# Renmusxd/RustQIP

Measured on AMD Instinct MI355X. Metric: single-qubit gate apply GB/s (algorithmic bytes: 32 * 2^n per H / X / Rz gate), higher is better.
Workload: dtype f64; 1 GPU; 256 random single-qubit gates (uniform H / X / Rz(theta), uniform target; configs[1] generator, seed 28, single-qubit part) at n=30 (30 qubits = 16 GiB per GPU), Complex<f64>, resident non-uniform state; n_qubits=30, n_local=30, parallelism=single GPU

## Files before the change

### rustqip_amd/build.py

```python
from __future__ import annotations

import os
import subprocess
import sys

HERE = os.path.dirname(os.path.abspath(__file__))
CSRC = os.path.join(HERE, "csrc")
UNITS = ["qip_core", "qip_launch", "qip_tile_sched", "qip_circuit", "qip_tile_interp", "qip_jit", "qip_slice", "qip_host", "qip_measure", "qip_dist"]
HEADERS = [os.path.join(CSRC, h) for h in ("qip_kernels.h", "qip_internal.h", "qip_jit.h", "qip_tile.h")] + [
    os.path.join(HERE, "..", "include", "qip_hip.h"), os.path.join(HERE, "..", "include", "qip_hip_debug.h"),
    os.path.join(HERE, "..", "include", "qip_hipx.h")]
OBJDIR = os.path.join(HERE, "build")
OUT = os.path.join(HERE, "lib", "libqip_hip.so")
JITC = os.path.join(HERE, "lib", "qip_jitc")
JITC_SRC = os.path.join(CSRC, "qip_jitc.c")
HIPCC = os.environ.get("HIPCC", "/opt/rocm/bin/hipcc")
FLAGS = ["--offload-arch=gfx950", "-O3", "-std=c++17", "-ffp-contract=off", "-fno-slp-vectorize", "-fPIC"]
if os.environ.get("QIP_HIP_TUNING"):
    FLAGS.append("-DQIP_HIP_TUNING")
UNIT_FLAGS = {"qip_tile_interp": ["-mllvm", "-structurizecfg-skip-uniform-regions"]}
LINK = ["--offload-arch=gfx950", "-fPIC", "-shared", "-Wl,--version-script=" + os.path.join(CSRC, "exports.map")]
LIBS = ["-ldl"]

EMBED = os.path.join(CSRC, "qip_kernels_embed.inc")


def write_embed() -> None:
    with open(HEADERS[0]) as f:
        text = f.read()
    assert ')QIPKSRC"' not in text
    body = 'R"QIPKSRC(' + text + ')QIPKSRC"\n'
    if not os.path.exists(EMBED) or open(EMBED).read() != body:
# ... 50 lines not shown
```

### rustqip_amd/csrc/qip_circuit.hip

```cpp
#include "qip_tile.h"

typedef std::complex<double> cd;
struct Cluster {
  std::vector<uint32_t> pos;
  std::vector<cd> m;
};

template <typename T>
static bool op_to_dense(uint32_t n, const FlatOp& f, uint32_t max_k, std::vector<uint32_t>* pos,
                        std::vector<cd>* mat) {
  if (!f.distinct || f.k_all > max_k) return false;
  const uint32_t kt = f.k_all, k = f.n_op;
  const size_t S = (size_t)1 << kt, Si = (size_t)1 << k, thr = S - Si;
  pos->clear();
  for (uint32_t j = 0; j < kt; ++j) pos->push_back(n - 1 - (uint32_t)f.outer->indices[j]);
  mat->assign(S * S, cd(0, 0));
  for (size_t r = 0; r < thr; ++r) (*mat)[r * S + r] = cd(1, 0);
  const T* dense = static_cast<const T*>(f.inner->dense);
  const T* vals = static_cast<const T*>(f.inner->sparse_vals);
  for (size_t r = 0; r < Si; ++r) {
    switch (f.inner->kind) {
      case QIP_OP_MATRIX:
        for (size_t c = 0; c < Si; ++c)
          (*mat)[(thr + r) * S + thr + c] = cd(dense[2 * (r * Si + c)], dense[2 * (r * Si + c) + 1]);
// ... 696 lines not shown
  if (run.prepare()) return QIP_OK;
  if (!params.empty()) QCHK(arena_upload(s, params.data(), params.size() * sizeof(T), 0));
  ProfRec rec;
  rec.cls = KC_TILE_GATES;
  if (s->profile) QCHK(prof_begin(s, KC_TILE_GATES, sweep_bytes, &rec));
  void* st_ptr = s->cur;
  uint64_t second_arg = ntiles;
  void* params_ptr = s->arena;
  void* out_ptr = s->alt;
  void* args_p[] = {&st_ptr, &second_arg, &params_ptr, &out_ptr};
  void* args_np[] = {&st_ptr, &second_arg, &out_ptr};
  void** args = (parametrised || !f.folding) ? args_p : args_np;
  const dim3 grid = grid2d(ntiles >> (f.sl ? f.sl->nbits : 0), 1);
  return run_parts(s, run, f, &rec, [&](uint32_t k) -> int {
    if (f.sl) second_arg = f.slice_or(k);
    return jit_run(s, job, [&](hipFunction_t fn) -> int {
      HIPCHK(hipModuleLaunchKernel(fn, grid.x, grid.y, 1, block, 1, 1, (unsigned)lds, s->stream, args, nullptr));
      return QIP_OK;
    });
  });
}

template <typename T>
static int launch_tile_segment(qip_hip_state* s, const BatchRun& run, const std::vector<const TileItem*>& seg,
                               std::vector<uint32_t> high_in, const TileStorePerm* fold = nullptr, TileSlicing* sl = nullptr,
                               uint32_t p5_override = 0, const std::vector<uint32_t>* grid_ctl = nullptr, double alg_bytes = 0) {
  arena_begin_group(s);
  TileSegmentPlan<T> plan;
  TileAbsorbedX absorbed;
  if (s->tile_passes && !run.tile_jit && !grid_ctl && !p5_override)
    QCHK(build_tile_segment_absorbed<T>(s->n, seg, std::move(high_in), &plan, run.tile >= 2 ? 2 : 1, &absorbed));
  else
    QCHK(build_tile_segment<T>(s->n, s->tile_passes != 0, seg, std::move(high_in), &plan, run.tile >= 2 ? 2 : 1, p5_override));
  const std::vector<uint32_t>& high = plan.high;
  TileInterpPlan<T> interp;
  if (!s->tile_passes && !plan.diags.empty()) return fail(QIP_ERR_INVALID, "internal: a multi-qubit diagonal item in a k_tile_gates segment");
  const bool use_runs = (g_tile_diag_runs || !plan.diags.empty()) && s->tile_passes && !run.tile_jit;
  if (use_runs) tile_merge_diag_runs<T>(plan, &interp, g_tile_diag_runs ? 2u : ~0u);
  const bool has_runs = use_runs && interp.runs > 0;
  std::vector<TileGate<T>>& gates = has_runs ? interp.gates : plan.gates;
  std::vector<amp_t<T>>& mats = plan.mats;
  TilePassDesc& pd = has_runs ? interp.pd : plan.pd;
  const size_t gates_bytes = gates.size() * sizeof(TileGate<T>);
  const size_t mats_bytes = mats.size() * sizeof(amp_t<T>);
  const size_t items_bytes = has_runs ? interp.items.size() * sizeof(TileDiagItem<T>) : 0;
  static_assert(sizeof(TileGate<T>) % 16 == 0, "the matrix block behind the gate list stays 16-byte aligned");
  static_assert(sizeof(amp_t<T>) * 16 % 16 == 0 && sizeof(TileDiagItem<T>) % 16 == 0, "... and the diagonal steps behind the matrices");
  const size_t items_off = (gates_bytes + mats_bytes + 15) / 16 * 16;
  auto upload_gates = [&]() -> int {
    QCHK(ensure_arena(s, items_off + items_bytes));
    QCHK(arena_upload(s, gates.data(), gates_bytes, 0));
    if (!mats.empty()) QCHK(arena_upload(s, mats.data(), mats_bytes, gates_bytes));
    if (items_bytes) QCHK(arena_upload(s, interp.items.data(), items_bytes, items_off));
    return QIP_OK;
  };
  TileDesc d;
  memset(&d, 0, sizeof d);
  d.ngates = (uint32_t)gates.size();
  for (int j = 0; j < kTileHigh; ++j) d.hpos[j] = high[j];
  d.p5 = plan.p5;
  Ins ins = tile_ins(high, plan.p5);
  uint64_t ntiles = 1ull << (s->n - kTileBits);
  const bool whole_grid = !grid_ctl || grid_ctl->empty();
  if (!whole_grid) {
    uint64_t ones = 0;
    for (uint32_t c : *grid_ctl) ones |= 1ull << (c == 5u ? plan.p5 : c);
    ins = tile_ins(high, plan.p5, *grid_ctl, ones);
    ntiles >>= grid_ctl->size();
  }
  const double sweep_bytes = alg_bytes > 0 ? alg_bytes : 2.0 * (double)s->amp_bytes * (double)s->namps;
  TileSweep f;
  QCHK(plan_sweep(s, run, fold, sl, s->tile_passes && whole_grid, kTileBits, high, plan.p5, &ins, &f));
  const size_t lds = sizeof(amp_t<T>) << kTileBits;
  if (s->tile_passes && run.tile_jit) {
    const bool fma = s->tile_fma && run.tile >= 2;
    const bool parametrised = run.tile_jit != 3;
// ... 2 lines not shown
    int remap = ntiles % 64 == 0 ? (int)g_tile_remap : 0;
    if (remap == 4) {
      uint32_t nb = 0, J = 0;
      while ((1ull << nb) < ntiles) ++nb;
      uint32_t seen = 0;
      for (uint32_t pp = kTileLow; pp < s->n && seen < nb; ++pp) {
        bool opened = false;
        for (uint32_t j = 0; j < ins.npos; ++j) opened = opened || ins.pos[j] == pp;
        if (opened) continue;
        if (pp < 16) ++J;
        ++seen;
      }
      if (nb < 3) remap = 0;
      else remap = 16 + (int)std::min(J, nb - 3);
    }
    if (f.sl) remap = 0;
    const std::string src = tile_jit_source<T>(plan, ins, use_nt(s), remap, parametrised ? &params : nullptr, merge, f.folding ? fold : nullptr, f.sl != nullptr);
    return launch_compiled<T>(s, run, f, src, fma, parametrised, params, ntiles, kTileBlock, lds, sweep_bytes);
  }
  if (run.prepare()) return QIP_OK;
  QCHK(upload_gates());
  const TileGate<T>* dg = (const TileGate<T>*)s->arena;
  const amp_t<T>* dmats = (const amp_t<T>*)((const char*)s->arena + gates_bytes);
  const TileDiagItem<T>* ditems = (const TileDiagItem<T>*)((const char*)s->arena + items_off);
  ProfRec rec;
  rec.cls = KC_TILE_GATES;
  if (s->profile) QCHK(prof_begin(s, KC_TILE_GATES, sweep_bytes, &rec));
  if (s->tile_passes) {
    const uint64_t ntiles_part = ntiles >> (f.sl ? f.sl->nbits : 0);
    return run_parts(s, run, f, &rec, [&](uint32_t k) -> int {
      Ins ins_k = ins;
      ins_k.ormask |= f.slice_or(k);
      launch_tile_passes<T>(s->stream, grid2d(ntiles_part, 1), lds, use_nt(s), (amp_t<T>*)s->cur, ins_k, pd, dg, dmats, (amp_t<T>*)s->alt,
                            f.folding ? fold : nullptr, ditems);
      HIPCHK(hipGetLastError());
      return QIP_OK;
    });
  }
  if (use_nt(s))
    hipLaunchKernelGGL((k_tile_gates<T, true>), grid2d(ntiles, 1), dim3(kBlock), lds, s->stream, (amp_t<T>*)s->cur, ins, d, dg);
  else
    hipLaunchKernelGGL((k_tile_gates<T, false>), grid2d(ntiles, 1), dim3(kBlock), lds, s->stream, (amp_t<T>*)s->cur, ins, d, dg);
  HIPCHK(hipGetLastError());
  if (s->profile) QCHK(prof_end(s, &rec));
  return QIP_OK;
}

template <typename T>
static int launch_wide_segment(qip_hip_state* s, const BatchRun& run, const std::vector<const TileItem*>& seg, std::vector<uint32_t> high_in,
                               const TileStorePerm* fold = nullptr, TileSlicing* sl = nullptr) {
  arena_begin_group(s);
  WidePlan<T> plan;
  QCHK(build_wide_segment<T>(s->n, seg, std::move(high_in), &plan, run.tile >= 2 ? 2 : 1));
  Ins ins = tile_ins(plan.high, plan.p5);
  TileSweep f;
  QCHK(plan_sweep(s, run, fold, sl, true, kWideBits, plan.high, plan.p5, &ins, &f));
// ... 681 lines not shown
```

### rustqip_amd/csrc/qip_kernels.h

```cpp
#pragma once

#ifndef __HIPCC_RTC__
#include <hip/hip_runtime.h>
#include <stdint.h>
#else
typedef __hip_internal::uint32_t uint32_t;
typedef __hip_internal::uint64_t uint64_t;
typedef __hip_internal::int32_t int32_t;
typedef __hip_internal::int64_t int64_t;
#endif

namespace qipk {

constexpr int kBlock = 256;
constexpr int kMaxIns = 64;

template <typename T> struct V2;
template <> struct V2<double> { using type = double __attribute__((ext_vector_type(2))); };
template <> struct V2<float> { using type = float __attribute__((ext_vector_type(2))); };
template <typename T> using amp_t = typename V2<T>::type;
template <typename A, typename B> struct SameT { static constexpr bool v = false; };
template <typename A> struct SameT<A, A> { static constexpr bool v = true; };
template <int V> struct IntC { static constexpr int v = V; };


struct Ins {
  uint64_t ormask;
  uint32_t npos;
  uint32_t pos[kMaxIns];
};

template <int NP>
// ... 1408 lines not shown
  for (int i = 0; i < NE; ++i) {
    if ((i >> J) & 1) continue;
    const int k = i | (1 << J);
    const A a0 = e[i], a1 = e[k];
    const T p0x = m0 * a0.x, p0y = m0 * a0.y, p1x = m1 * a1.x, p1y = m1 * a1.y;
    e[i].x = p0x + p1x;
    e[i].y = p0y + p1y;
    e[k].x = tile_signed_sum<N0, N1>(p0x, p1x);
    e[k].y = tile_signed_sum<N0, N1>(p0y, p1y);
    __builtin_amdgcn_sched_barrier(0);
  }
}

template <typename T, int J, int NE>
__device__ __forceinline__ void pass_dense_signs(const TileGate<T>& g, amp_t<T> (&e)[NE]) {
  switch (g.b1 & (kTileSignNeg0 | kTileSignNeg1)) {
    case 0u: pass_dense_signs_body<T, J, false, false, NE>(g, e); break;
    case kTileSignNeg1: pass_dense_signs_body<T, J, false, true, NE>(g, e); break;
    case kTileSignNeg0: pass_dense_signs_body<T, J, true, false, NE>(g, e); break;
    default: pass_dense_signs_body<T, J, true, true, NE>(g, e); break;
  }
}

template <typename T, int J, int NE, bool LOOP = false>
__device__ __forceinline__ void pass_dense(const TileGate<T>& g, amp_t<T> (&e)[NE], const uint32_t (&c)[NE], uint32_t cm) {
  using A = amp_t<T>;
  const bool is_x = (g.b1 & 2u) != 0, real = (g.b1 & 1u) != 0;
  if (is_x) {
#pragma unroll
    for (int i = 0; i < NE; ++i) {
      if ((i >> J) & 1) continue;
      const int k = i | (1 << J);
      if ((c[i] & cm) != cm) continue;
      QIP_KEEP_BRANCH();
      if constexpr (LOOP) {
        cswap_inplace(e[i], e[k]);
      } else {
        const A a0 = e[i];
        e[i] = e[k];
        e[k] = a0;
      }
    }
    return;
  }
  if (cm == 0u && real && (g.b1 & kTileSignRows) != 0) {
    QIP_KEEP_BRANCH();
    pass_dense_signs<T, J, NE>(g, e);
  } else if (cm == 0u && g.nz == 15u) {
    if (real) pass_dense_body<T, J, true, false, NE, LOOP>(g, e, c, cm);
    else pass_dense_body<T, J, false, false, NE, LOOP>(g, e, c, cm);
  } else {
    if (real) pass_dense_body<T, J, true, true, NE, LOOP>(g, e, c, cm);
    else pass_dense_body<T, J, false, true, NE, LOOP>(g, e, c, cm);
  }
}

template <typename T, int J, int NE>
__device__ __forceinline__ void pass_dense_lane(const TileGate<T>& g, amp_t<T> (&e)[NE], const uint32_t (&c)[NE], uint32_t cm,
                                                bool lane_ok) {
  using A = amp_t<T>;
  const bool h0 = (g.nz & 1u) != 0, h1 = (g.nz & 2u) != 0, h2 = (g.nz & 4u) != 0, h3 = (g.nz & 8u) != 0;
#pragma unroll
  for (int i = 0; i < NE; ++i) {
    if ((i >> J) & 1) continue;
    const int k = i | (1 << J);
    if ((c[i] & cm) != cm) continue;
    QIP_KEEP_BRANCH();
    const A a0 = e[i], a1 = e[k];
// ... 99 lines not shown
    if (((base >> JA) & 1) || ((base >> JB) & 1) || ((base >> JC) & 1)) continue;
    if ((c[base] & cm) != cm) continue;
    QIP_KEEP_BRANCH();
    A x[8];
#pragma unroll
    for (int s = 0; s < 8; ++s) x[s] = e[base | (((s >> 2) & 1) << JA) | (((s >> 1) & 1) << JB) | ((s & 1) << JC)];
#pragma unroll
    for (int r = 0; r < 8; ++r) {
      A acc = cmul(M[r * 8], x[0]);
#pragma unroll
      for (int s = 1; s < 8; ++s) acc = cadd(acc, cmul(M[r * 8 + s], x[s]));
      const int i = base | (((r >> 2) & 1) << JA) | (((r >> 1) & 1) << JB) | ((r & 1) << JC);
      e[i] = lane_ctl ? tile_sel(lane_ok, acc, x[r]) : acc;
      __builtin_amdgcn_sched_barrier(0);
    }
  }
}
template <typename T, int JA, int JB, int JC>
__device__ __forceinline__ void pass_dense3(const amp_t<T>* __restrict__ M, amp_t<T> (&e)[8], bool lane_ctl, bool lane_ok) {
  const uint32_t c0[8] = {0, 0, 0, 0, 0, 0, 0, 0};
  pass_dense3w<T, JA, JB, JC, 8>(M, e, c0, 0u, lane_ctl, lane_ok);
}

template <typename T, bool NT, bool FOLD = false>
__global__ __launch_bounds__(kTileBlock, 5) void k_tile_passes(amp_t<T>* __restrict__ st, Ins ins, TilePassDesc d,
                                                                              const TileGate<T>* __restrict__ gates,
                                                                              const amp_t<T>* __restrict__ mats,
                                                                              amp_t<T>* __restrict__ out = nullptr,
                                                                              TileStorePerm sp = TileStorePerm(),
                                                                              const TileDiagItem<T>* __restrict__ diag = nullptr) {
  using A = amp_t<T>;
  extern __shared__ __attribute__((aligned(16))) unsigned char tile_raw[];
  A* tile = reinterpret_cast<A*>(tile_raw);
  constexpr int PER = (1 << kTileBits) / kTileBlock;
  static_assert(PER == 8 && kTileLow == 6, "tile index = (u << kTileLaneBits) | (wave << 6) | lane");
  const uint32_t tid = threadIdx.x;
  const uint32_t lane = tid & 63u;
  const uint32_t wave = __builtin_amdgcn_readfirstlane(tid >> 6);
  uint64_t wbase = tile_block_base(blockIdx.x + (uint64_t)blockIdx.y * gridDim.x, ins, d.p5);
  const uint64_t base = wbase;
#pragma unroll
  for (int j = 0; j < kTileWaveBits; ++j) wbase |= (uint64_t)((wave >> j) & 1u) << d.hpos[j];
  const uint32_t slot_tid = tile_slot<A>(tid);
  const uint32_t lane_off = tile_lane_off(lane, d.p5);
  {
    A x[PER];
#pragma unroll
    for (int u = 0; u < PER; ++u) {
      const uint64_t ub = wbase | ((uint64_t)(u & 1) << d.hpos[kTileWaveBits]) | ((uint64_t)((u >> 1) & 1) << d.hpos[kTileWaveBits + 1]) |
                          ((uint64_t)((u >> 2) & 1) << d.hpos[kTileWaveBits + 2]);
      x[u] = ldg<NT>(st + ub + lane_off);
    }
#pragma unroll
    for (int u = 0; u < PER; ++u) tile[slot_tid ^ tile_slot<A>((uint32_t)u << kTileLaneBits)] = x[u];
  }
  __syncthreads();
  for (uint32_t pi = 0; pi < d.npasses; ++pi) {
    const TilePass ps = d.pass[pi];
    uint32_t tb = 0;
    const uint32_t lp_lo = (uint32_t)ps.lanepos, lp_hi = (uint32_t)(ps.lanepos >> 32);
#pragma unroll
    for (int k = 0; k < kTileLaneBits; ++k) tb |= ((tid >> k) & 1u) << (((k < 8 ? lp_lo : lp_hi) >> (4 * (k & 7))) & 15u);
    const uint32_t slot_tb = tile_slot<A>(tb);
    uint32_t c[8];
    A e[8];
#pragma unroll
    for (int i = 0; i < 8; ++i) {
      c[i] = ((uint32_t)(i & 1) << ps.pb[0]) | ((uint32_t)((i >> 1) & 1) << ps.pb[1]) |
             ((uint32_t)((i >> 2) & 1) << ps.pb[2]);
      e[i] = tile[slot_tb ^ tile_slot<A>(c[i])];
    }
    const TileGate<T>* gp = gates + ps.first;
    const TileGate<T>* const gend = gp + ps.count;
    for (; gp != gend; ++gp) {
      const TileGate<T> g = *gp;
      if ((base & g.omask) != g.omask) continue;
      const uint32_t cm_reg = g.cm_reg;
      switch (g.op) {
        case TOP_DIAG_RUN: {
          const TileDiagItem<T>* ip = diag + g.nz;
          const TileDiagItem<T>* const iend = ip + g.b1;
#ifndef QIP_DIAG_PREFETCH
#define QIP_DIAG_PREFETCH 0
#endif
#ifndef QIP_DIAG_ASM
#define QIP_DIAG_ASM 1
#endif
#if QIP_DIAG_PREFETCH
          TileDiagItem<T> nxt = *ip;
#endif
          for (; ip != iend;) {
#if QIP_DIAG_PREFETCH
            const TileDiagItem<T> it = nxt;
            ++ip;
            if (ip != iend) nxt = *ip;
#else
            const TileDiagItem<T> it = *ip;
            ++ip;
#endif
            if ((base & it.omask) != it.oval) continue;
            A f = it.f1;
            const uint32_t selp = it.emask_sel >> 24;
            if (selp != 0u) {
              QIP_KEEP_BRANCH();
              f = tile_sel(((tb >> (selp - 1u)) & 1u) != 0u, it.f1, it.f0);
            }
            if (it.lane_mask != 0u) {
              QIP_KEEP_BRANCH();
              const bool lane_ok = (tb & it.lane_mask) == it.lane_val;
              f.x = lane_ok ? f.x : (T)1;
              f.y = lane_ok ? f.y : (T)0;
            }
#pragma unroll
            for (int i = 0; i < 8; ++i)
              if ((it.emask_sel >> i) & 1u) {
                QIP_KEEP_BRANCH();
#if QIP_DIAG_ASM
                cscale_inplace(f, e[i]);
#else
                e[i] = cmul(f, e[i]);
#endif
              }
          }
          break;
        }
        case TOP_DIAG_UNIFORM: {
          const A f = ((base >> g.tpos_out) & 1ull) ? g.m[1] : g.m[0];
          if (f.x == (T)1 && f.y == (T)0) break;
          QIP_KEEP_BRANCH();
          pass_scale<T, 0, -1, 8, true>(f, e, c, cm_reg);
          break;
        }
        case TOP_DIAG_LANE:
        case TOP_DIAG_LANE_CTL: {
          const bool outside = g.b0 == kTileOutside;
          const bool one = outside ? ((base >> g.tpos_out) & 1ull) != 0 : ((tb >> g.b0) & 1u) != 0;
          A f = tile_sel(one, g.m[1], g.m[0]);
          if (g.op == TOP_DIAG_LANE_CTL) {
            QIP_KEEP_BRANCH();
            const bool lane_ok = (tb & g.cm_lane) == g.cm_lane;
            f.x = lane_ok ? f.x : (T)1;
            f.y = lane_ok ? f.y : (T)0;
          }
          pass_scale<T, 0, -1, 8, true>(f, e, c, cm_reg);
          break;
        }
        case TOP_DIAG_REG0: pass_diag<T, 0, 8, true>(g, e, c, cm_reg, g.cm_lane != 0u, (tb & g.cm_lane) == g.cm_lane); break;
        case TOP_DIAG_REG1: pass_diag<T, 1, 8, true>(g, e, c, cm_reg, g.cm_lane != 0u, (tb & g.cm_lane) == g.cm_lane); break;
        case TOP_DIAG_REG2: pass_diag<T, 2, 8, true>(g, e, c, cm_reg, g.cm_lane != 0u, (tb & g.cm_lane) == g.cm_lane); break;
        case TOP_DENSE0: pass_dense<T, 0, 8, true>(g, e, c, cm_reg); break;
        case TOP_DENSE1: pass_dense<T, 1, 8, true>(g, e, c, cm_reg); break;
        case TOP_DENSE2: pass_dense<T, 2, 8, true>(g, e, c, cm_reg); break;
        case TOP_DENSE_LANE0: pass_dense_lane<T, 0>(g, e, c, cm_reg, (tb & g.cm_lane) == g.cm_lane); break;
        case TOP_DENSE_LANE1: pass_dense_lane<T, 1>(g, e, c, cm_reg, (tb & g.cm_lane) == g.cm_lane); break;
        case TOP_DENSE_LANE2: pass_dense_lane<T, 2>(g, e, c, cm_reg, (tb & g.cm_lane) == g.cm_lane); break;
#define QIP_D2Q(JA, JB) \
  pass_dense2<T, JA, JB>(mats + 16u * g.nz, e, c, cm_reg, g.cm_lane != 0u, (tb & g.cm_lane) == g.cm_lane)
        case TOP_DENSE2Q_01: QIP_D2Q(0, 1); break;
        case TOP_DENSE2Q_02: QIP_D2Q(0, 2); break;
        case TOP_DENSE2Q_10: QIP_D2Q(1, 0); break;
        case TOP_DENSE2Q_12: QIP_D2Q(1, 2); break;
        case TOP_DENSE2Q_20: QIP_D2Q(2, 0); break;
        case TOP_DENSE2Q_21: QIP_D2Q(2, 1); break;
#undef QIP_D2Q
        case TOP_SWAP_01: pass_swap<T, 0, 1, 8, true>(e, c, cm_reg, g.cm_lane != 0u, (tb & g.cm_lane) == g.cm_lane); break;
        case TOP_SWAP_02: pass_swap<T, 0, 2, 8, true>(e, c, cm_reg, g.cm_lane != 0u, (tb & g.cm_lane) == g.cm_lane); break;
        case TOP_SWAP_12: pass_swap<T, 1, 2, 8, true>(e, c, cm_reg, g.cm_lane != 0u, (tb & g.cm_lane) == g.cm_lane); break;
#define QIP_D3Q(JA, JB, JC) pass_dense3<T, JA, JB, JC>(mats + 16u * g.nz, e, g.cm_lane != 0u, (tb & g.cm_lane) == g.cm_lane)
        case TOP_DENSE3Q_012: QIP_D3Q(0, 1, 2); break;
        case TOP_DENSE3Q_021: QIP_D3Q(0, 2, 1); break;
        case TOP_DENSE3Q_102: QIP_D3Q(1, 0, 2); break;
        case TOP_DENSE3Q_120: QIP_D3Q(1, 2, 0); break;
        case TOP_DENSE3Q_201: QIP_D3Q(2, 0, 1); break;
        case TOP_DENSE3Q_210: QIP_D3Q(2, 1, 0); break;
#undef QIP_D3Q
        default: break;
      }
    }
#pragma unroll
    for (int i = 0; i < 8; ++i) tile[slot_tb ^ tile_slot<A>(c[i])] = e[i];
    __syncthreads();
  }
  {
    const uint32_t slot_src = slot_tid ^ tile_slot<A>(d.flip & ((1u << kTileBits) - 1u));
#pragma unroll
    for (int u = 0; u < PER; ++u) {
      const uint64_t ub = wbase | ((uint64_t)(u & 1) << d.hpos[kTileWaveBits]) | ((uint64_t)((u >> 1) & 1) << d.hpos[kTileWaveBits + 1]) |
                          ((uint64_t)((u >> 2) & 1) << d.hpos[kTileWaveBits + 2]);
      if constexpr (FOLD) stg<NT>(out + tile_packed_index(ub, sp) + tile_packed_index(lane_off, sp), tile[slot_src ^ tile_slot<A>((uint32_t)u << kTileLaneBits)]);
      else stg<NT>(st + ub + lane_off, tile[slot_src ^ tile_slot<A>((uint32_t)u << kTileLaneBits)]);
    }
  }
}

struct TileMfmaDesc {
  uint32_t hpos[kTileHigh];
  uint32_t tb[5];
  uint32_t nb[kTileBits - 4];
  uint32_t p5;
};

template <typename T, int K, bool NT, bool LOOP, int NP>
__global__ __launch_bounds__(kTileBlock, K == 4 ? 5 : 2) void k_gate_tile_mfma(amp_t<T>* __restrict__ st, Ins ins, TileMfmaDesc d,
                                                                              const T* __restrict__ afrag, uint32_t pipe) {
  const uint32_t PIPE = LOOP ? pipe : 1u;
  using A = amp_t<T>;
  using V4 = typename Acc4<T>::type;
  constexpr int S = 1 << K, TT = S / 8, KS = S / 2, NA = S / 4;
  constexpr int IB = kTileBits - K - 4;
  constexpr int IPW = (1 << IB) / (kTileBlock / 64);
  static_assert(IPW >= 1 && TT % 2 == 0, "tile shape");
  extern __shared__ __attribute__((aligned(16))) unsigned char tile_raw[];
  A* tile = reinterpret_cast<A*>(tile_raw);
  const uint32_t tid = threadIdx.x, lane = tid & 63u;
  const uint32_t wave = __builtin_amdgcn_readfirstlane(tid >> 6);
  const uint64_t first = (blockIdx.x + (uint64_t)blockIdx.y * gridDim.x) * PIPE;
// ... 1374 lines not shown
```

### rustqip_amd/csrc/qip_tile.h

```cpp
#pragma once
#include "qip_internal.h"

struct TileItem {
  bool tileable = false;
  bool exact = false;
  int kind = 0;
  std::vector<uint32_t> pos;
  uint32_t t0 = 0, t1 = 0, t2 = 0;
  std::vector<uint32_t> cpos;
  double m[8] = {0};
  uint32_t nz = 0;
  std::vector<double> mat;
  uint32_t dk = 0;
  uint64_t nd_mask = 0, d_mask = 0;
  std::vector<std::pair<uint32_t, uint32_t>> swap_pairs;
};
constexpr int kTileKindDiagK = 5;
constexpr uint32_t kTopDiagItem = (uint32_t)TOP_DIAG_RUN + 1u;
static inline bool tile_item_is_diag(const TileItem& it) { return it.kind == 1 || it.kind == kTileKindDiagK; }
static inline bool tile_item_needs_passes(const TileItem& it) { return it.kind == 3 || it.kind == 4 || it.kind == kTileKindDiagK; }
template <typename T> struct TileDiagSpec {
  uint32_t k;
  uint32_t bit[3];
  uint32_t pos[3];
// ... 40 lines not shown
  return it.kind == 0 ? 1 : it.kind == 2 || it.kind == 3 ? 2 : it.kind == 4 ? 3 : 0;
}

template <typename T> struct TileSegmentPlan {
  std::vector<uint32_t> high;
  std::vector<TileGate<T>> gates;
  std::vector<amp_t<T>> mats;
  std::vector<TileDiagSpec<T>> diags;
  TilePassDesc pd;
  uint32_t p5 = 5;
  std::vector<uint32_t> order;
};

template <typename T> struct TileInterpPlan {
  std::vector<TileGate<T>> gates;
  std::vector<TileDiagItem<T>> items;
  TilePassDesc pd;
  uint32_t runs = 0, gates_in_runs = 0;
};
template <typename T> void tile_merge_diag_runs(const TileSegmentPlan<T>& plan, TileInterpPlan<T>* out, uint32_t min_run = 2);
extern int64_t g_tile_diag_runs;
template <typename T>
void launch_tile_passes(hipStream_t stream, dim3 grid, size_t lds, bool nt, amp_t<T>* st, const Ins& ins, const TilePassDesc& pd,
                        const TileGate<T>* gates, const amp_t<T>* mats, amp_t<T>* out, const TileStorePerm* fold,
                        const TileDiagItem<T>* items);

struct TileAbsorbedX {
  std::vector<const TileItem*> seg;
  std::deque<TileItem> owned;
  uint64_t flip = 0;
  uint32_t absorbed = 0;
};
void tile_absorb_x(const std::vector<const TileItem*>& seg, TileAbsorbedX* out);
template <typename T>
int build_tile_segment_absorbed(uint32_t n, const std::vector<const TileItem*>& seg, std::vector<uint32_t> high, TileSegmentPlan<T>* out,
                                int order_rule, TileAbsorbedX* ab);

struct TileStep {
  std::vector<uint64_t> ops;
  std::vector<uint32_t> high;
  std::vector<uint32_t> perm;
};

struct TileSchedule {
  const qip_op* circuit = nullptr;
  uint64_t count = 0;
  std::vector<qip_op> owned;
  std::deque<std::vector<uint64_t>> idx;
// ... 48 lines not shown
```

### rustqip_amd/csrc/qip_tile_interp.hip

```cpp
#include "qip_tile.h"

template <typename T>
void launch_tile_passes(hipStream_t stream, dim3 grid, size_t lds, bool nt, amp_t<T>* st, const Ins& ins, const TilePassDesc& pd,
                        const TileGate<T>* gates, const amp_t<T>* mats, amp_t<T>* out, const TileStorePerm* fold,
                        const TileDiagItem<T>* items) {
  if (fold) {
#define TPF(NTV) hipLaunchKernelGGL((k_tile_passes<T, NTV, true>), grid, dim3(kTileBlock), lds, stream, st, ins, pd, gates, mats, out, *fold, items)
    if (nt) TPF(true);
    else TPF(false);
#undef TPF
  } else {
#define TP(NTV) hipLaunchKernelGGL((k_tile_passes<T, NTV>), grid, dim3(kTileBlock), lds, stream, st, ins, pd, gates, mats, (amp_t<T>*)nullptr, TileStorePerm(), items)
    if (nt) TP(true);
    else TP(false);
#undef TP
  }
}
template void launch_tile_passes<double>(hipStream_t, dim3, size_t, bool, amp_t<double>*, const Ins&, const TilePassDesc&, const TileGate<double>*,
                                         const amp_t<double>*, amp_t<double>*, const TileStorePerm*, const TileDiagItem<double>*);
template void launch_tile_passes<float>(hipStream_t, dim3, size_t, bool, amp_t<float>*, const Ins&, const TilePassDesc&, const TileGate<float>*,
                                        const amp_t<float>*, amp_t<float>*, const TileStorePerm*, const TileDiagItem<float>*);
```

Measured before the change: 98940 GB/s.

## Pack tile gate and diagonal items into 64-byte wire format with scalar fetch

Adds a compact wire encoding for tile-pass gates and diagonal run items, aligned to 64-byte blocks and loaded as one 16-dword scalar vector. Gate dispatch uses precomputed codes, including dedicated sign-row dense ops. Diagonal items carry a form byte so common element masks map to specialized scale passes, and complementary lo/hi item pairs are merged into one. The aim is to cut per-gate scalar load and decode cost in the interpreter loop. The trade-offs are larger padded records, host-side packing, and extra kernel branches.

```diff
diff --git a/rustqip_amd/build.py b/rustqip_amd/build.py
--- a/rustqip_amd/build.py
+++ b/rustqip_amd/build.py
@@ -7,7 +7,7 @@
 HERE = os.path.dirname(os.path.abspath(__file__))
 CSRC = os.path.join(HERE, "csrc")
 UNITS = ["qip_core", "qip_launch", "qip_tile_sched", "qip_circuit", "qip_tile_interp", "qip_jit", "qip_slice", "qip_host", "qip_measure", "qip_dist"]
-HEADERS = [os.path.join(CSRC, h) for h in ("qip_kernels.h", "qip_internal.h", "qip_jit.h", "qip_tile.h")] + [
+HEADERS = [os.path.join(CSRC, h) for h in ("qip_kernels.h", "qip_internal.h", "qip_jit.h", "qip_tile.h", "qip_tile_wire.h")] + [
     os.path.join(HERE, "..", "include", "qip_hip.h"), os.path.join(HERE, "..", "include", "qip_hip_debug.h"),
     os.path.join(HERE, "..", "include", "qip_hipx.h")]
 OBJDIR = os.path.join(HERE, "build")
diff --git a/rustqip_amd/csrc/qip_circuit.hip b/rustqip_amd/csrc/qip_circuit.hip
--- a/rustqip_amd/csrc/qip_circuit.hip
+++ b/rustqip_amd/csrc/qip_circuit.hip
@@ -742,6 +742,28 @@
 }
 
 template <typename T>
+static int tile_wire_pack(const std::vector<TileGate<T>>& gates, const std::vector<TileDiagItem<T>>& items, std::vector<TileWireGate<T>>* wg,
+                          std::vector<TileWireItem<T>>* wi) {
+  const TileWireOps ops = {TOP_DIAG_UNIFORM, TOP_DIAG_LANE, TOP_DIAG_LANE_CTL, TOP_DENSE0, TOP_DIAG_RUN};
+  wg->resize(gates.size());
+  wi->resize(items.size());
+  size_t n = 0;
+  for (size_t i = 0; i < gates.size(); ++i) {
+    const TileGate<T>& g = gates[i];
+    if (!wire_pack_gate<T>(g, ops, &(*wg)[i])) return fail(QIP_ERR_INVALID, "internal: a tile gate field does not fit the wire format");
+    if (g.op != TOP_DIAG_RUN) continue;
+    if ((size_t)g.nz + g.b1 > items.size()) return fail(QIP_ERR_INVALID, "internal: a diagonal run beyond the item list");
+    const long k = wire_pack_items<T>(items.data() + g.nz, g.b1, wi->data() + n);
+    if (k < 0) return fail(QIP_ERR_INVALID, "internal: a diagonal item field does not fit the wire format");
+    (*wg)[i].nz = (uint32_t)n;
+    (*wg)[i].b1 = (uint32_t)k;
+    n += (size_t)k;
+  }
+  wi->resize(n);
+  return QIP_OK;
+}
+
+template <typename T>
 static int launch_tile_segment(qip_hip_state* s, const BatchRun& run, const std::vector<const TileItem*>& seg,
                                std::vector<uint32_t> high_in, const TileStorePerm* fold = nullptr, TileSlicing* sl = nullptr,
                                uint32_t p5_override = 0, const std::vector<uint32_t>* grid_ctl = nullptr, double alg_bytes = 0) {
@@ -761,17 +783,21 @@
   std::vector<TileGate<T>>& gates = has_runs ? interp.gates : plan.gates;
   std::vector<amp_t<T>>& mats = plan.mats;
   TilePassDesc& pd = has_runs ? interp.pd : plan.pd;
-  const size_t gates_bytes = gates.size() * sizeof(TileGate<T>);
+  const bool wire = s->tile_passes && !run.tile_jit;
+  std::vector<TileWireGate<T>> wgates;
+  std::vector<TileWireItem<T>> witems;
+  if (wire) QCHK(tile_wire_pack<T>(gates, interp.items, &wgates, &witems));
+  const size_t gates_bytes = wire ? wgates.size() * sizeof(TileWireGate<T>) : gates.size() * sizeof(TileGate<T>);
   const size_t mats_bytes = mats.size() * sizeof(amp_t<T>);
-  const size_t items_bytes = has_runs ? interp.items.size() * sizeof(TileDiagItem<T>) : 0;
-  static_assert(sizeof(TileGate<T>) % 16 == 0, "the matrix block behind the gate list stays 16-byte aligned");
-  static_assert(sizeof(amp_t<T>) * 16 % 16 == 0 && sizeof(TileDiagItem<T>) % 16 == 0, "... and the diagonal steps behind the matrices");
-  const size_t items_off = (gates_bytes + mats_bytes + 15) / 16 * 16;
+  const size_t items_bytes = has_runs ? witems.size() * sizeof(TileWireItem<T>) : 0;
+  static_assert(sizeof(TileGate<T>) % 16 == 0 && sizeof(TileWireGate<T>) % 64 == 0, "the matrix block behind the gate list stays 16-byte aligned");
+  static_assert(sizeof(amp_t<T>) * 16 % 16 == 0 && sizeof(TileWireItem<T>) == 64, "... and the diagonal steps behind the matrices, on a block boundary");
+  const size_t items_off = (gates_bytes + mats_bytes + 63) / 64 * 64;
   auto upload_gates = [&]() -> int {
     QCHK(ensure_arena(s, items_off + items_bytes));
-    QCHK(arena_upload(s, gates.data(), gates_bytes, 0));
+    QCHK(arena_upload(s, wire ? (const void*)wgates.data() : (const void*)gates.data(), gates_bytes, 0));
     if (!mats.empty()) QCHK(arena_upload(s, mats.data(), mats_bytes, gates_bytes));
-    if (items_bytes) QCHK(arena_upload(s, interp.items.data(), items_bytes, items_off));
+    if (items_bytes) QCHK(arena_upload(s, witems.data(), items_bytes, items_off));
     return QIP_OK;
   };
   TileDesc d;
@@ -820,7 +846,8 @@
   QCHK(upload_gates());
   const TileGate<T>* dg = (const TileGate<T>*)s->arena;
   const amp_t<T>* dmats = (const amp_t<T>*)((const char*)s->arena + gates_bytes);
-  const TileDiagItem<T>* ditems = (const TileDiagItem<T>*)((const char*)s->arena + items_off);
+  const TileWireGate<T>* wg = (const TileWireGate<T>*)s->arena;
+  const TileWireItem<T>* ditems = (const TileWireItem<T>*)((const char*)s->arena + items_off);
   ProfRec rec;
   rec.cls = KC_TILE_GATES;
   if (s->profile) QCHK(prof_begin(s, KC_TILE_GATES, sweep_bytes, &rec));
@@ -829,7 +856,7 @@
     return run_parts(s, run, f, &rec, [&](uint32_t k) -> int {
       Ins ins_k = ins;
       ins_k.ormask |= f.slice_or(k);
-      launch_tile_passes<T>(s->stream, grid2d(ntiles_part, 1), lds, use_nt(s), (amp_t<T>*)s->cur, ins_k, pd, dg, dmats, (amp_t<T>*)s->alt,
+      launch_tile_passes<T>(s->stream, grid2d(ntiles_part, 1), lds, use_nt(s), (amp_t<T>*)s->cur, ins_k, pd, wg, dmats, (amp_t<T>*)s->alt,
                             f.folding ? fold : nullptr, ditems);
       HIPCHK(hipGetLastError());
       return QIP_OK;
diff --git a/rustqip_amd/csrc/qip_kernels.h b/rustqip_amd/csrc/qip_kernels.h
--- a/rustqip_amd/csrc/qip_kernels.h
+++ b/rustqip_amd/csrc/qip_kernels.h
@@ -8,6 +8,10 @@
 typedef __hip_internal::uint64_t uint64_t;
 typedef __hip_internal::int32_t int32_t;
 typedef __hip_internal::int64_t int64_t;
+#endif
+
+#ifndef __HIPCC_RTC__
+#include "qip_tile_wire.h"
 #endif
 
 namespace qipk {
@@ -1462,7 +1466,7 @@
   }
 }
 
-template <typename T, int J, int NE, bool LOOP = false>
+template <typename T, int J, int NE, bool LOOP = false, bool SIGNS = true>
 __device__ __forceinline__ void pass_dense(const TileGate<T>& g, amp_t<T> (&e)[NE], const uint32_t (&c)[NE], uint32_t cm) {
   using A = amp_t<T>;
   const bool is_x = (g.b1 & 2u) != 0, real = (g.b1 & 1u) != 0;
@@ -1483,7 +1487,7 @@
     }
     return;
   }
-  if (cm == 0u && real && (g.b1 & kTileSignRows) != 0) {
+  if (SIGNS && cm == 0u && real && (g.b1 & kTileSignRows) != 0) {
     QIP_KEEP_BRANCH();
     pass_dense_signs<T, J, NE>(g, e);
   } else if (cm == 0u && g.nz == 15u) {
@@ -1629,13 +1633,36 @@
   pass_dense3w<T, JA, JB, JC, 8>(M, e, c0, 0u, lane_ctl, lane_ok);
 }
 
+#ifndef __HIPCC_RTC__
+static_assert(kTileBits == (int)kWireTileBits && kMaxIns <= (int)kWireMaxPos && kTileMaxGates == (int)kWireMaxGates,
+              "qip_tile_wire.h: the bounds its narrow fields are sized for");
+typedef uint32_t wire_words_t __attribute__((ext_vector_type(16)));
+__device__ __forceinline__ wire_words_t wire_fetch(const void* __restrict__ p) {
+  wire_words_t w = *reinterpret_cast<const wire_words_t*>(p);
+  asm volatile("" : "+s"(w));
+  return w;
+}
+__device__ __forceinline__ uint64_t wire_u64(uint32_t lo, uint32_t hi) { return (uint64_t)lo | ((uint64_t)hi << 32); }
+__device__ __forceinline__ float wire_f32(uint32_t u) { return __builtin_bit_cast(float, u); }
+template <typename T, int W> __device__ __forceinline__ amp_t<T> wire_amp(const wire_words_t& w) {
+  amp_t<T> a;
+  if constexpr (sizeof(T) == 8) {
+    a.x = __builtin_bit_cast(double, wire_u64(w[W], w[W + 1]));
+    a.y = __builtin_bit_cast(double, wire_u64(w[W + 2], w[W + 3]));
+  } else {
+    a.x = wire_f32(w[W]);
+    a.y = wire_f32(w[W + 1]);
+  }
+  return a;
+}
+
 template <typename T, bool NT, bool FOLD = false>
 __global__ __launch_bounds__(kTileBlock, 5) void k_tile_passes(amp_t<T>* __restrict__ st, Ins ins, TilePassDesc d,
-                                                                              const TileGate<T>* __restrict__ gates,
+                                                                              const TileWireGate<T>* __restrict__ gates,
                                                                               const amp_t<T>* __restrict__ mats,
                                                                               amp_t<T>* __restrict__ out = nullptr,
                                                                               TileStorePerm sp = TileStorePerm(),
-                                                                              const TileDiagItem<T>* __restrict__ diag = nullptr) {
+                                                                              const TileWireItem<T>* __restrict__ diag = nullptr) {
   using A = amp_t<T>;
   extern __shared__ __attribute__((aligned(16))) unsigned char tile_raw[];
   A* tile = reinterpret_cast<A*>(tile_raw);
@@ -1677,110 +1704,156 @@
              ((uint32_t)((i >> 2) & 1) << ps.pb[2]);
       e[i] = tile[slot_tb ^ tile_slot<A>(c[i])];
     }
-    const TileGate<T>* gp = gates + ps.first;
-    const TileGate<T>* const gend = gp + ps.count;
+    using WW = TileWireWords<T>;
+    const TileWireGate<T>* gp = gates + ps.first;
+    const TileWireGate<T>* const gend = gp + ps.count;
     for (; gp != gend; ++gp) {
-      const TileGate<T> g = *gp;
-      if ((base & g.omask) != g.omask) continue;
-      const uint32_t cm_reg = g.cm_reg;
-      switch (g.op) {
-        case TOP_DIAG_RUN: {
-          const TileDiagItem<T>* ip = diag + g.nz;
-          const TileDiagItem<T>* const iend = ip + g.b1;
-#ifndef QIP_DIAG_PREFETCH
-#define QIP_DIAG_PREFETCH 0
-#endif
-#ifndef QIP_DIAG_ASM
-#define QIP_DIAG_ASM 1
-#endif
-#if QIP_DIAG_PREFETCH
-          TileDiagItem<T> nxt = *ip;
-#endif
+      const wire_words_t w = wire_fetch(gp);
+      const uint64_t omask = wire_u64(w[kWireWOmask], w[kWireWOmask + 1]);
+      if ((base & omask) != omask) continue;
+      const uint32_t cm_reg = wire_cm_reg(w[kWireWCm]), cm_lane = wire_cm_lane(w[kWireWCm]);
+      auto gate_of = [&](auto full) {
+        TileGate<T> g;
+        g.b1 = w[kWireWB1];
+        g.nz = w[kWireWNz];
+        g.m[0] = wire_amp<T, WW::m0>(w);
+        g.m[1] = wire_amp<T, WW::m1>(w);
+        if constexpr (decltype(full)::v != 0) {
+          if constexpr (sizeof(T) == 8) {
+            const amp_t<T>* __restrict__ m23 = reinterpret_cast<const amp_t<T>*>(gp->m23);
+            g.m[2] = m23[0];
+            g.m[3] = m23[1];
+          } else {
+            g.m[2] = wire_amp<T, WW::m2>(w);
+            g.m[3] = wire_amp<T, WW::m3>(w);
+          }
+        }
+        return g;
+      };
+      const uint32_t code = w[kWireWCode];
+      switch (code) {
+        case WOP_SIGNS0: pass_dense_signs<T, 0, 8>(gate_of(IntC<0>()), e); break;
+        case WOP_SIGNS1: pass_dense_signs<T, 1, 8>(gate_of(IntC<0>()), e); break;
+        case WOP_SIGNS2: pass_dense_signs<T, 2, 8>(gate_of(IntC<0>()), e); break;
+        case WOP_RUN: {
+          const TileWireItem<T>* ip = diag + w[kWireWNz];
+          const TileWireItem<T>* const iend = ip + w[kWireWB1];
           for (; ip != iend;) {
-#if QIP_DIAG_PREFETCH
-            const TileDiagItem<T> it = nxt;
+            const wire_words_t it = wire_fetch(ip);
             ++ip;
-            if (ip != iend) nxt = *ip;
-#else
-            const TileDiagItem<T> it = *ip;
-            ++ip;
-#endif
-            if ((base & it.omask) != it.oval) continue;
-            A f = it.f1;
-            const uint32_t selp = it.emask_sel >> 24;
+            if ((base & wire_u64(it[WW::omask], it[WW::omask + 1])) != wire_u64(it[WW::oval], it[WW::oval + 1])) continue;
+            const uint32_t ctl = it[WW::ctl], lane = it[WW::lane];
+            const uint32_t form = wire_form(ctl);
+            A f = wire_amp<T, WW::f1>(it);
+            if (form >= WF_BOTH0) {
+              QIP_KEEP_BRANCH();
+              A fl = wire_amp<T, WW::f0>(it);
+              if (lane != 0u) {
+                QIP_KEEP_BRANCH();
+                const bool lane_ok = (tb & wire_lane_mask(lane)) == wire_lane_val(lane);
+                fl.x = lane_ok ? fl.x : (T)1;
+                fl.y = lane_ok ? fl.y : (T)0;
+                f.x = lane_ok ? f.x : (T)1;
+                f.y = lane_ok ? f.y : (T)0;
+              }
+              if (form == WF_BOTH0) {
+                QIP_KEEP_BRANCH();
+                pass_scale<T, 0, 0, 8, true>(fl, e, c, 0u);
+                pass_scale<T, 0, 1, 8, true>(f, e, c, 0u);
+              } else if (form == WF_BOTH1) {
+                QIP_KEEP_BRANCH();
+                pass_scale<T, 1, 0, 8, true>(fl, e, c, 0u);
+                pass_scale<T, 1, 1, 8, true>(f, e, c, 0u);
+              } else {
+                QIP_KEEP_BRANCH();
+                pass_scale<T, 2, 0, 8, true>(fl, e, c, 0u);
+                pass_scale<T, 2, 1, 8, true>(f, e, c, 0u);
+              }
+              continue;
+            }
+            const uint32_t selp = wire_sel(ctl);
             if (selp != 0u) {
               QIP_KEEP_BRANCH();
-              f = tile_sel(((tb >> (selp - 1u)) & 1u) != 0u, it.f1, it.f0);
+              f = tile_sel(((tb >> (selp - 1u)) & 1u) != 0u, f, wire_amp<T, WW::f0>(it));
             }
-            if (it.lane_mask != 0u) {
+            if (lane != 0u) {
               QIP_KEEP_BRANCH();
-              const bool lane_ok = (tb & it.lane_mask) == it.lane_val;
+              const bool lane_ok = (tb & wire_lane_mask(lane)) == wire_lane_val(lane);
               f.x = lane_ok ? f.x : (T)1;
               f.y = lane_ok ? f.y : (T)0;
             }
-#pragma unroll
-            for (int i = 0; i < 8; ++i)
-              if ((it.emask_sel >> i) & 1u) {
-                QIP_KEEP_BRANCH();
-#if QIP_DIAG_ASM
-                cscale_inplace(f, e[i]);
-#else
-                e[i] = cmul(f, e[i]);
-#endif
-              }
+            switch (form) {
+              case WF_ALL: pass_scale<T, 0, -1, 8, true>(f, e, c, 0u); break;
+              case WF_LO0: pass_scale<T, 0, 0, 8, true>(f, e, c, 0u); break;
+              case WF_HI0: pass_scale<T, 0, 1, 8, true>(f, e, c, 0u); break;
+              case WF_LO1: pass_scale<T, 1, 0, 8, true>(f, e, c, 0u); break;
+              case WF_HI1: pass_scale<T, 1, 1, 8, true>(f, e, c, 0u); break;
+              case WF_LO2: pass_scale<T, 2, 0, 8, true>(f, e, c, 0u); break;
+              case WF_HI2: pass_scale<T, 2, 1, 8, true>(f, e, c, 0u); break;
+              default:
+#pragma unroll
+                for (int i = 0; i < 8; ++i)
+                  if ((ctl >> i) & 1u) {
+                    QIP_KEEP_BRANCH();
+                    cscale_inplace(f, e[i]);
+                  }
+                break;
+            }
           }
           break;
         }
-        case TOP_DIAG_UNIFORM: {
-          const A f = ((base >> g.tpos_out) & 1ull) ? g.m[1] : g.m[0];
+        case WOP_DIAG_UNIFORM: {
+          const A f = ((base >> wire_tpos_out(w[kWireWBits])) & 1ull) ? wire_amp<T, WW::m1>(w) : wire_amp<T, WW::m0>(w);
           if (f.x == (T)1 && f.y == (T)0) break;
           QIP_KEEP_BRANCH();
           pass_scale<T, 0, -1, 8, true>(f, e, c, cm_reg);
           break;
         }
-        case TOP_DIAG_LANE:
-        case TOP_DIAG_LANE_CTL: {
-          const bool outside = g.b0 == kTileOutside;
-          const bool one = outside ? ((base >> g.tpos_out) & 1ull) != 0 : ((tb >> g.b0) & 1u) != 0;
-          A f = tile_sel(one, g.m[1], g.m[0]);
-          if (g.op == TOP_DIAG_LANE_CTL) {
+        case WOP_DIAG_LANE: {
+          const uint32_t b0 = wire_b0(w[kWireWBits]);
+          const bool outside = b0 == kWireOutside;
+          const bool one = outside ? ((base >> wire_tpos_out(w[kWireWBits])) & 1ull) != 0 : ((tb >> b0) & 1u) != 0;
+          A f = tile_sel(one, wire_amp<T, WW::m1>(w), wire_amp<T, WW::m0>(w));
+          if (cm_lane != 0u) {
             QIP_KEEP_BRANCH();
-            const bool lane_ok = (tb & g.cm_lane) == g.cm_lane;
+            const bool lane_ok = (tb & cm_lane) == cm_lane;
             f.x = lane_ok ? f.x : (T)1;
             f.y = lane_ok ? f.y : (T)0;
           }
           pass_scale<T, 0, -1, 8, true>(f, e, c, cm_reg);
           break;
         }
-        case TOP_DIAG_REG0: pass_diag<T, 0, 8, true>(g, e, c, cm_reg, g.cm_lane != 0u, (tb & g.cm_lane) == g.cm_lane); break;
-        case TOP_DIAG_REG1: pass_diag<T, 1, 8, true>(g, e, c, cm_reg, g.cm_lane != 0u, (tb & g.cm_lane) == g.cm_lane); break;
-        case TOP_DIAG_REG2: pass_diag<T, 2, 8, true>(g, e, c, cm_reg, g.cm_lane != 0u, (tb & g.cm_lane) == g.cm_lane); break;
-        case TOP_DENSE0: pass_dense<T, 0, 8, true>(g, e, c, cm_reg); break;
-        case TOP_DENSE1: pass_dense<T, 1, 8, true>(g, e, c, cm_reg); break;
-        case TOP_DENSE2: pass_dense<T, 2, 8, true>(g, e, c, cm_reg); break;
-        case TOP_DENSE_LANE0: pass_dense_lane<T, 0>(g, e, c, cm_reg, (tb & g.cm_lane) == g.cm_lane); break;
-        case TOP_DENSE_LANE1: pass_dense_lane<T, 1>(g, e, c, cm_reg, (tb & g.cm_lane) == g.cm_lane); break;
-        case TOP_DENSE_LANE2: pass_dense_lane<T, 2>(g, e, c, cm_reg, (tb & g.cm_lane) == g.cm_lane); break;
+#define QIP_WOP(op) kWireOther + (uint32_t)(op)
+        case QIP_WOP(TOP_DIAG_REG0): pass_diag<T, 0, 8, true>(gate_of(IntC<0>()), e, c, cm_reg, cm_lane != 0u, (tb & cm_lane) == cm_lane); break;
+        case QIP_WOP(TOP_DIAG_REG1): pass_diag<T, 1, 8, true>(gate_of(IntC<0>()), e, c, cm_reg, cm_lane != 0u, (tb & cm_lane) == cm_lane); break;
+        case QIP_WOP(TOP_DIAG_REG2): pass_diag<T, 2, 8, true>(gate_of(IntC<0>()), e, c, cm_reg, cm_lane != 0u, (tb & cm_lane) == cm_lane); break;
+        case QIP_WOP(TOP_DENSE0): pass_dense<T, 0, 8, true, false>(gate_of(IntC<1>()), e, c, cm_reg); break;
+        case QIP_WOP(TOP_DENSE1): pass_dense<T, 1, 8, true, false>(gate_of(IntC<1>()), e, c, cm_reg); break;
+        case QIP_WOP(TOP_DENSE2): pass_dense<T, 2, 8, true, false>(gate_of(IntC<1>()), e, c, cm_reg); break;
+        case QIP_WOP(TOP_DENSE_LANE0): pass_dense_lane<T, 0>(gate_of(IntC<1>()), e, c, cm_reg, (tb & cm_lane) == cm_lane); break;
+        case QIP_WOP(TOP_DENSE_LANE1): pass_dense_lane<T, 1>(gate_of(IntC<1>()), e, c, cm_reg, (tb & cm_lane) == cm_lane); break;
+        case QIP_WOP(TOP_DENSE_LANE2): pass_dense_lane<T, 2>(gate_of(IntC<1>()), e, c, cm_reg, (tb & cm_lane) == cm_lane); break;
 #define QIP_D2Q(JA, JB) \
-  pass_dense2<T, JA, JB>(mats + 16u * g.nz, e, c, cm_reg, g.cm_lane != 0u, (tb & g.cm_lane) == g.cm_lane)
-        case TOP_DENSE2Q_01: QIP_D2Q(0, 1); break;
-        case TOP_DENSE2Q_02: QIP_D2Q(0, 2); break;
-        case TOP_DENSE2Q_10: QIP_D2Q(1, 0); break;
-        case TOP_DENSE2Q_12: QIP_D2Q(1, 2); break;
-        case TOP_DENSE2Q_20: QIP_D2Q(2, 0); break;
-        case TOP_DENSE2Q_21: QIP_D2Q(2, 1); break;
+  pass_dense2<T, JA, JB>(mats + 16u * w[kWireWNz], e, c, cm_reg, cm_lane != 0u, (tb & cm_lane) == cm_lane)
+        case QIP_WOP(TOP_DENSE2Q_01): QIP_D2Q(0, 1); break;
+        case QIP_WOP(TOP_DENSE2Q_02): QIP_D2Q(0, 2); break;
+        case QIP_WOP(TOP_DENSE2Q_10): QIP_D2Q(1, 0); break;
+        case QIP_WOP(TOP_DENSE2Q_12): QIP_D2Q(1, 2); break;
+        case QIP_WOP(TOP_DENSE2Q_20): QIP_D2Q(2, 0); break;
+        case QIP_WOP(TOP_DENSE2Q_21): QIP_D2Q(2, 1); break;
 #undef QIP_D2Q
-        case TOP_SWAP_01: pass_swap<T, 0, 1, 8, true>(e, c, cm_reg, g.cm_lane != 0u, (tb & g.cm_lane) == g.cm_lane); break;
-        case TOP_SWAP_02: pass_swap<T, 0, 2, 8, true>(e, c, cm_reg, g.cm_lane != 0u, (tb & g.cm_lane) == g.cm_lane); break;
-        case TOP_SWAP_12: pass_swap<T, 1, 2, 8, true>(e, c, cm_reg, g.cm_lane != 0u, (tb & g.cm_lane) == g.cm_lane); break;
-#define QIP_D3Q(JA, JB, JC) pass_dense3<T, JA, JB, JC>(mats + 16u * g.nz, e, g.cm_lane != 0u, (tb & g.cm_lane) == g.cm_lane)
-        case TOP_DENSE3Q_012: QIP_D3Q(0, 1, 2); break;
-        case TOP_DENSE3Q_021: QIP_D3Q(0, 2, 1); break;
-        case TOP_DENSE3Q_102: QIP_D3Q(1, 0, 2); break;
-        case TOP_DENSE3Q_120: QIP_D3Q(1, 2, 0); break;
-        case TOP_DENSE3Q_201: QIP_D3Q(2, 0, 1); break;
-        case TOP_DENSE3Q_210: QIP_D3Q(2, 1, 0); break;
+        case QIP_WOP(TOP_SWAP_01): pass_swap<T, 0, 1, 8, true>(e, c, cm_reg, cm_lane != 0u, (tb & cm_lane) == cm_lane); break;
+        case QIP_WOP(TOP_SWAP_02): pass_swap<T, 0, 2, 8, true>(e, c, cm_reg, cm_lane != 0u, (tb & cm_lane) == cm_lane); break;
+        case QIP_WOP(TOP_SWAP_12): pass_swap<T, 1, 2, 8, true>(e, c, cm_reg, cm_lane != 0u, (tb & cm_lane) == cm_lane); break;
+#define QIP_D3Q(JA, JB, JC) pass_dense3<T, JA, JB, JC>(mats + 16u * w[kWireWNz], e, cm_lane != 0u, (tb & cm_lane) == cm_lane)
+        case QIP_WOP(TOP_DENSE3Q_012): QIP_D3Q(0, 1, 2); break;
+        case QIP_WOP(TOP_DENSE3Q_021): QIP_D3Q(0, 2, 1); break;
+        case QIP_WOP(TOP_DENSE3Q_102): QIP_D3Q(1, 0, 2); break;
+        case QIP_WOP(TOP_DENSE3Q_120): QIP_D3Q(1, 2, 0); break;
+        case QIP_WOP(TOP_DENSE3Q_201): QIP_D3Q(2, 0, 1); break;
+        case QIP_WOP(TOP_DENSE3Q_210): QIP_D3Q(2, 1, 0); break;
 #undef QIP_D3Q
+#undef QIP_WOP
         default: break;
       }
     }
@@ -1799,6 +1872,7 @@
     }
   }
 }
+#endif
 
 struct TileMfmaDesc {
   uint32_t hpos[kTileHigh];
diff --git a/rustqip_amd/csrc/qip_tile.h b/rustqip_amd/csrc/qip_tile.h
--- a/rustqip_amd/csrc/qip_tile.h
+++ b/rustqip_amd/csrc/qip_tile.h
@@ -86,8 +86,8 @@
 extern int64_t g_tile_diag_runs;
 template <typename T>
 void launch_tile_passes(hipStream_t stream, dim3 grid, size_t lds, bool nt, amp_t<T>* st, const Ins& ins, const TilePassDesc& pd,
-                        const TileGate<T>* gates, const amp_t<T>* mats, amp_t<T>* out, const TileStorePerm* fold,
-                        const TileDiagItem<T>* items);
+                        const TileWireGate<T>* gates, const amp_t<T>* mats, amp_t<T>* out, const TileStorePerm* fold,
+                        const TileWireItem<T>* items);
 
 struct TileAbsorbedX {
   std::vector<const TileItem*> seg;
diff --git a/rustqip_amd/csrc/qip_tile_interp.hip b/rustqip_amd/csrc/qip_tile_interp.hip
--- a/rustqip_amd/csrc/qip_tile_interp.hip
+++ b/rustqip_amd/csrc/qip_tile_interp.hip
@@ -2,8 +2,8 @@
 
 template <typename T>
 void launch_tile_passes(hipStream_t stream, dim3 grid, size_t lds, bool nt, amp_t<T>* st, const Ins& ins, const TilePassDesc& pd,
-                        const TileGate<T>* gates, const amp_t<T>* mats, amp_t<T>* out, const TileStorePerm* fold,
-                        const TileDiagItem<T>* items) {
+                        const TileWireGate<T>* gates, const amp_t<T>* mats, amp_t<T>* out, const TileStorePerm* fold,
+                        const TileWireItem<T>* items) {
   if (fold) {
 #define TPF(NTV) hipLaunchKernelGGL((k_tile_passes<T, NTV, true>), grid, dim3(kTileBlock), lds, stream, st, ins, pd, gates, mats, out, *fold, items)
     if (nt) TPF(true);
@@ -16,7 +16,7 @@
 #undef TP
   }
 }
-template void launch_tile_passes<double>(hipStream_t, dim3, size_t, bool, amp_t<double>*, const Ins&, const TilePassDesc&, const TileGate<double>*,
-                                         const amp_t<double>*, amp_t<double>*, const TileStorePerm*, const TileDiagItem<double>*);
-template void launch_tile_passes<float>(hipStream_t, dim3, size_t, bool, amp_t<float>*, const Ins&, const TilePassDesc&, const TileGate<float>*,
-                                        const amp_t<float>*, amp_t<float>*, const TileStorePerm*, const TileDiagItem<float>*);
+template void launch_tile_passes<double>(hipStream_t, dim3, size_t, bool, amp_t<double>*, const Ins&, const TilePassDesc&, const TileWireGate<double>*,
+                                         const amp_t<double>*, amp_t<double>*, const TileStorePerm*, const TileWireItem<double>*);
+template void launch_tile_passes<float>(hipStream_t, dim3, size_t, bool, amp_t<float>*, const Ins&, const TilePassDesc&, const TileWireGate<float>*,
+                                        const amp_t<float>*, amp_t<float>*, const TileStorePerm*, const TileWireItem<float>*);
diff --git a/rustqip_amd/csrc/qip_tile_wire.h b/rustqip_amd/csrc/qip_tile_wire.h
--- /dev/null
+++ b/rustqip_amd/csrc/qip_tile_wire.h
@@ -0,0 +1,144 @@
+#pragma once
+#include <stdint.h>
+
+#if defined(__HIPCC__)
+#define QIP_WIRE_HD __host__ __device__ __forceinline__
+#else
+#define QIP_WIRE_HD inline
+#endif
+
+namespace qipk {
+
+constexpr uint32_t kWireTileBits = 11;
+constexpr uint32_t kWireMaxPos = 64;
+constexpr uint32_t kWireMaxGates = 256;
+constexpr uint32_t kWireItemsPerGate = 8;
+constexpr uint32_t kWireOutside = 0xffu;
+static_assert(kWireTileBits <= 16, "cm_reg, cm_lane, lane_mask, lane_val: 16 bits each");
+static_assert(kWireTileBits < kWireOutside && kWireMaxPos <= 256, "b0 (or the outside mark) and tpos_out: 8 bits each");
+static_assert(kWireMaxGates * kWireItemsPerGate < (1u << 24), "a run's first item and item count: below the form byte");
+
+enum TileWireOp : uint32_t {
+  WOP_SIGNS0 = 0, WOP_SIGNS1, WOP_SIGNS2,
+  WOP_RUN,
+  WOP_DIAG_UNIFORM,
+  WOP_DIAG_LANE,
+  kWireOther = 8,
+};
+
+enum TileWireForm : uint32_t {
+  WF_MASK = 0,
+  WF_ALL,
+  WF_LO0, WF_HI0, WF_LO1, WF_HI1, WF_LO2, WF_HI2,
+  WF_BOTH0, WF_BOTH1, WF_BOTH2,
+};
+
+template <typename T> struct TileWireGate;
+template <> struct alignas(64) TileWireGate<double> {
+  uint32_t code, b1, nz, cm, bits, pad_;
+  uint64_t omask;
+  double m01[4];
+  double m23[4];
+  uint32_t pad1_[8];
+};
+template <> struct alignas(64) TileWireGate<float> {
+  uint32_t code, b1, nz, cm, bits, pad_;
+  uint64_t omask;
+  float m01[4];
+  float m23[4];
+};
+static_assert(sizeof(TileWireGate<double>) == 128 && sizeof(TileWireGate<float>) == 64, "one / two 64-byte blocks");
+
+template <typename T> struct alignas(64) TileWireItem {
+  T f0[2], f1[2];
+  uint64_t omask, oval;
+  uint32_t lane;
+  uint32_t ctl;
+};
+static_assert(sizeof(TileWireItem<double>) == 64 && sizeof(TileWireItem<float>) == 64, "one 64-byte block per run item");
+
+constexpr int kWireWCode = 0, kWireWB1 = 1, kWireWNz = 2, kWireWCm = 3, kWireWBits = 4, kWireWOmask = 6, kWireWM = 8;
+QIP_WIRE_HD uint32_t wire_cm_reg(uint32_t cm) { return cm & 0xffffu; }
+QIP_WIRE_HD uint32_t wire_cm_lane(uint32_t cm) { return cm >> 16; }
+QIP_WIRE_HD uint32_t wire_b0(uint32_t bits) { return bits & 0xffu; }
+QIP_WIRE_HD uint32_t wire_tpos_out(uint32_t bits) { return bits >> 8; }
+template <typename T> struct TileWireWords {
+  static constexpr int amp = (int)sizeof(T) / 2;
+  static constexpr int m0 = kWireWM, m1 = kWireWM + amp, m2 = kWireWM + 2 * amp, m3 = kWireWM + 3 * amp;
+  static constexpr int f0 = 0, f1 = amp, omask = 2 * amp, oval = 2 * amp + 2, lane = 2 * amp + 4, ctl = 2 * amp + 5;
+};
+QIP_WIRE_HD uint32_t wire_lane_mask(uint32_t lane) { return lane & 0xffffu; }
+QIP_WIRE_HD uint32_t wire_lane_val(uint32_t lane) { return lane >> 16; }
+QIP_WIRE_HD uint32_t wire_emask(uint32_t ctl) { return ctl & 0xffu; }
+QIP_WIRE_HD uint32_t wire_form(uint32_t ctl) { return (ctl >> 8) & 0xffu; }
+QIP_WIRE_HD uint32_t wire_sel(uint32_t ctl) { return ctl >> 16; }
+
+struct TileWireOps {
+  uint32_t diag_uniform, diag_lane, diag_lane_ctl, dense0, diag_run;
+};
+template <typename T, typename G> inline bool wire_pack_gate(const G& g, const TileWireOps& ops, TileWireGate<T>* w) {
+  *w = TileWireGate<T>();
+  const bool outside = g.b0 == 0xffffffffu;
+  if ((!outside && g.b0 >= kWireOutside) || g.tpos_out >= (1u << 24) || g.cm_reg > 0xffffu || g.cm_lane > 0xffffu) return false;
+  uint32_t code = kWireOther + g.op;
+  if (g.op >= ops.dense0 && g.op < ops.dense0 + 3u && (g.b1 & 2u) == 0u && (g.b1 & 1u) != 0u && (g.b1 & 4u) != 0u && g.cm_reg == 0u)
+    code = WOP_SIGNS0 + (g.op - ops.dense0);
+  else if (g.op == ops.diag_run) code = WOP_RUN;
+  else if (g.op == ops.diag_uniform) code = WOP_DIAG_UNIFORM;
+  else if (g.op == ops.diag_lane || g.op == ops.diag_lane_ctl) code = WOP_DIAG_LANE;
+  w->code = code;
+  w->b1 = g.b1;
+  w->nz = g.nz;
+  w->cm = g.cm_reg | ((g.op == ops.diag_lane ? 0u : g.cm_lane) << 16);
+  w->bits = (outside ? kWireOutside : g.b0) | (g.tpos_out << 8);
+  w->omask = g.omask;
+  for (int k = 0; k < 2; ++k) {
+    w->m01[2 * k] = g.m[k].x;
+    w->m01[2 * k + 1] = g.m[k].y;
+    w->m23[2 * k] = g.m[2 + k].x;
+    w->m23[2 * k + 1] = g.m[2 + k].y;
+  }
+  return true;
+}
+
+inline uint32_t wire_form_of(uint32_t emask) {
+  static const uint32_t lo[3] = {0x55u, 0x33u, 0x0fu};
+  if (emask == 0xffu) return WF_ALL;
+  for (uint32_t j = 0; j < 3; ++j) {
+    if (emask == lo[j]) return WF_LO0 + 2u * j;
+    if (emask == (lo[j] ^ 0xffu)) return WF_HI0 + 2u * j;
+  }
+  return WF_MASK;
+}
+
+template <typename T, typename I> inline long wire_pack_items(const I* items, uint32_t count, TileWireItem<T>* out) {
+  long n = 0;
+  for (uint32_t k = 0; k < count; ++k) {
+    const I& a = items[k];
+    const uint32_t emask = a.emask_sel & 0xffu, sel = a.emask_sel >> 24;
+    if (a.lane_mask > 0xffffu || a.lane_val > 0xffffu || (a.emask_sel & 0x00ffff00u) != 0u) return -1;
+    TileWireItem<T> w = TileWireItem<T>();
+    w.f0[0] = a.f0.x, w.f0[1] = a.f0.y, w.f1[0] = a.f1.x, w.f1[1] = a.f1.y;
+    w.omask = a.omask;
+    w.oval = a.oval;
+    w.lane = a.lane_mask | (a.lane_val << 16);
+    uint32_t form = wire_form_of(emask);
+    if (sel == 0u && form >= WF_LO0 && form <= WF_HI2 && k + 1 < count) {
+      const I& b = items[k + 1];
+      const bool lo_first = ((form - WF_LO0) & 1u) == 0u;
+      if ((b.emask_sel >> 24) == 0u && (b.emask_sel & 0xffu) == (emask ^ 0xffu) && b.omask == a.omask && b.oval == a.oval &&
+          b.lane_mask == a.lane_mask && b.lane_val == a.lane_val) {
+        const I& lo = lo_first ? a : b;
+        const I& hi = lo_first ? b : a;
+        w.f0[0] = lo.f1.x, w.f0[1] = lo.f1.y, w.f1[0] = hi.f1.x, w.f1[1] = hi.f1.y;
+        form = WF_BOTH0 + (form - WF_LO0) / 2u;
+        ++k;
+      }
+    }
+    w.ctl = (form == WF_BOTH0 || form == WF_BOTH1 || form == WF_BOTH2 ? 0xffu : emask) | (form << 8) | (sel << 16);
+    out[n++] = w;
+  }
+  return n;
+}
+
+}
```

After: 100,000 GB/s, median of 6. 1.01x the previous value.
